# aperezhortal/pySPEEDY

Measured on AMD Instinct MI355X. Metric: simulated-years/day (whole node), T30L8, higher is better.
Workload: dtype f64

## Files before the change

### pyspeedy_amd/csrc/dynamics.hip

```cpp
#include <hip/hip_runtime.h>

#include <type_traits>

#include "coupler_point.hpp"
#include "device_tables.hpp"
#include "diagnostics_block.hpp"
#include "dyn_column.hpp"
#include "launch_events.hpp"
#include "model.hpp"
#include "sppt_point.hpp"

namespace spd {

namespace {
using d2 = double __attribute__((ext_vector_type(2)));
constexpr int NG = IX * IL;
constexpr int kT = 256;

__device__ constexpr double CPd = 1004.0f;
__device__ constexpr double AKAPd = 2.0f / 7.0f;
__device__ constexpr double RGASd = AKAPd * CPd;
__device__ constexpr double WILd = 0.53f, TDRSd = 24.0f * 30.0f;

__device__ inline d2 times_i(d2 z) { return d2{-z.y, z.x}; }
__device__ inline d2 operator_scale(double c, d2 z) { return d2{c * z.x, c * z.y}; }

struct Stencil {
    d2 ac, bc, ap, bp, an, bn;
};
__device__ inline Stencil load_stencil(const d2 *a, const d2 *b, int k, int n) {
    const int kp = n > 0 ? k - MX : k, kn = n < NX - 1 ? k + MX : k;
    return Stencil{a[k], b[k], a[kp], b[kp], a[kn], b[kn]};
}
template <int MODE>
__device__ inline void apply_stencil(const Stencil &s, int k, int m, int n, const DeviceTables &T, d2 &ra, d2 &rb) {
    const double *tym = MODE == 0 ? T.uvdym : T.vddym, *typ = MODE == 0 ? T.uvdyp : T.vddyp;
    const double dx = MODE == 0 ? T.uvdx[k] : T.gradx[m];
    const double cm = tym[k], cp = typ[k];
    const d2 zp = times_i(d2{dx * s.ac.x, dx * s.ac.y}), zc = times_i(d2{dx * s.bc.x, dx * s.bc.y});
    if (n == 0) {
        ra = d2{zc.x - cp * s.an.x, zc.y - cp * s.an.y};
        rb = d2{zp.x + cp * s.bn.x, zp.y + cp * s.bn.y};
    } else if (n == NX - 1) {
        ra = d2{cm * s.ap.x, cm * s.ap.y};
        rb = d2{-cm * s.bp.x, -cm * s.bp.y};
    } else {
        ra = d2{cm * s.ap.x - cp * s.an.x + zc.x, cm * s.ap.y - cp * s.an.y + zc.y};
        rb = d2{-cm * s.bp.x + cp * s.bn.x + zp.x, -cm * s.bp.y + cp * s.bn.y + zp.y};
    }
}
}

namespace {
__device__ __forceinline__ d2 geo_up(d2 ph_below, d2 t_below, d2 t_here, double xg2_below, double xg1_here) {
    return d2{fma(xg1_here, t_here.x, fma(xg2_below, t_below.x, ph_below.x)),
              fma(xg1_here, t_here.y, fma(xg2_below, t_below.y, ph_below.y))};
}
__device__ __forceinline__ d2 geo_corr(d2 ph, d2 t_below, d2 t_above, double corf) {
    return d2{fma(corf, t_below.x - t_above.x, ph.x), fma(corf, t_below.y - t_above.y, ph.y)};
}
}

template <bool SPPT>
__global__ __launch_bounds__(kT) void geopotential_kernel(ModelPtrs P, DynDeviceTables D, int first, int count, int tl, SpptArgs sp) {
    const int ngeo = (count * NSPEC + kT - 1) / kT;
    if (SPPT && static_cast<int>(blockIdx.x) >= ngeo) {
        sppt_update_point(sp, static_cast<long>(blockIdx.x - ngeo) * kT + threadIdx.x);
        return;
    }
    const int gid = blockIdx.x * kT + threadIdx.x;
    if (gid >= count * NSPEC) return;
    const int lm = gid / NSPEC, mem = first + lm, k = gid - lm * NSPEC, m = k % MX;
    const d2 *t = reinterpret_cast<const d2 *>(P.t) + (static_cast<size_t>(mem) * 2 + tl) * 8 * NSPEC + k;
    d2 *phi = reinterpret_cast<d2 *>(P.phi) + static_cast<size_t>(mem) * 8 * NSPEC + k;
    d2 tt[KX], ph[KX];
#pragma unroll
    for (int l = 0; l < KX; ++l) tt[l] = t[static_cast<size_t>(l) * NSPEC];
    const d2 phis = reinterpret_cast<const d2 *>(P.phis)[static_cast<size_t>(mem) * NSPEC + k];
    ph[KX - 1] = d2{fma(D.xgeop1[KX - 1], tt[KX - 1].x, phis.x), fma(D.xgeop1[KX - 1], tt[KX - 1].y, phis.y)};
#pragma unroll
    for (int l = KX - 2; l >= 0; --l) ph[l] = geo_up(ph[l + 1], tt[l + 1], tt[l], D.xgeop2[l + 1], D.xgeop1[l]);
    if (m == 0) {
#pragma unroll
        for (int l = 1; l < KX - 1; ++l) ph[l] = geo_corr(ph[l], tt[l + 1], tt[l - 1], D.geo_corf[l]);
    }
#pragma unroll
    for (int l = 0; l < KX; ++l) phi[static_cast<size_t>(l) * NSPEC] = ph[l];
}

__global__ __launch_bounds__(kT) void dyn_grid_kernel(ModelPtrs P, DynDeviceTables D, int M) {
    const int gid = blockIdx.x * kT + threadIdx.x;
    if (gid >= M * NG) return;
    const int mem = gid / NG, p = gid - mem * NG, j = p / IX;
    double ttend[KX], trtend[KX], ut, vt;
    dyn_column<true>(P, D, mem, p, j, ttend, trtend, ut, vt);
}

namespace {
constexpr int kCoefBlocks = NSPEC / 8;
static_assert(NSPEC % 8 == 0, "coefficient blocks");

__device__ inline void gather_levels(d2 v, int kk, d2 (&out)[KX]) {
#pragma unroll
    for (int l = 0; l < KX; ++l) out[l] = d2{__shfl(v.x, 8 * l + kk), __shfl(v.y, 8 * l + kk)};
}
template <int N>
__device__ inline double pick(const double (&a)[N], int l) {
    double r = a[0];
#pragma unroll
    for (int i = 1; i < N; ++i) r = (l == i) ? a[i] : r;
    return r;
}
template <int N>
__device__ inline d2 pick(const d2 (&a)[N], int l) {
    d2 r = a[0];
#pragma unroll
    for (int i = 1; i < N; ++i) r = (l == i) ? a[i] : r;
    return r;
}
}

struct NoCoupler {};
template <bool FOLD, bool EARLY, typename CA>
__global__ __launch_bounds__(kT) void spectral_step_kernel(ModelPtrs P, DeviceTables T, DynDeviceTables D, int M, int first,
                                                           int count, int j1, double dt, double eps, CA cpl) {
    int nblocks = gridDim.x;
    if constexpr (std::is_same<CA, CouplerArgs>::value) {
        nblocks = (count * NSPEC * KX + kT - 1) / kT;
        if (static_cast<int>(blockIdx.x) >= nblocks) {
            const int gid = (blockIdx.x - nblocks) * kT + threadIdx.x;
            if (gid < cpl.count * NG) {
                const int lm = gid / NG;
                coupler_point(cpl.S, cpl.first + lm, gid - lm * NG, cpl.w, cpl.day, cpl.land_coupling, cpl.sst_anomaly,
                              cpl.anom_planes, cpl.fresh);
            }
            return;
        }
    }
    const int xcd = blockIdx.x & 7, q = nblocks >> 3, r = nblocks & 7;
    const int block = xcd * q + (xcd < r ? xcd : r) + (blockIdx.x >> 3);
    const int gid = block * kT + threadIdx.x;
    const int w = gid >> 6, lane = gid & 63;
    if (w >= count * kCoefBlocks) return;
    const int l = lane >> 3, kk = lane & 7;
    const int lm = w / kCoefBlocks, mem = first + lm, k = (w - lm * kCoefBlocks) * 8 + kk, n = k / MX, m = k - n * MX;
    const size_t f8 = static_cast<size_t>(mem) * 8 * NSPEC;
    const size_t pair = static_cast<size_t>(M) * 8 * NSPEC;
    const size_t fo = static_cast<size_t>(l) * NSPEC;
    const d2 *su = reinterpret_cast<const d2 *>(P.specu) + f8 + fo, *sv = reinterpret_cast<const d2 *>(P.specv) + f8 + fo;
    const double el2 = T.el2[k];
    d2 vordt, divdt, tdt, trdt, dump;
    const size_t s0 = static_cast<size_t>(mem) * 2 * 8 * NSPEC + fo + k;
    const size_t lvl = static_cast<size_t>(8) * NSPEC;
    d2 *vorS = reinterpret_cast<d2 *>(P.vor) + s0, *divS = reinterpret_cast<d2 *>(P.div) + s0;
    d2 *tS = reinterpret_cast<d2 *>(P.t) + s0, *trS = reinterpret_cast<d2 *>(P.tr) + s0;
    d2 *psS = reinterpret_cast<d2 *>(P.ps) + static_cast<size_t>(mem) * 2 * NSPEC + k;
    const int l_tot = m + n;
    d2 ke, stt, str, psdt, ph, div1, ps1;
    d2 vor1, t1, tr1, tcorh, qcorh, phis_k{0.0, 0.0}, vor2{}, div2{}, t2{}, tr2{}, ps2{};
    double xc_l[KX], xj_l[KX], xd_l[KX], elz, dmp, dmp1, dmpd, dmp1d, dmps, dmp1s, trf;
    auto load_diffusion = [&]() {
        dmp = D.dmp[k], dmp1 = D.dmp1[k], dmpd = D.dmpd[k], dmp1d = D.dmp1d[k], dmps = D.dmps[k], dmp1s = D.dmp1s[k];
        trf = T.trfilt[k];
        tcorh = reinterpret_cast<const d2 *>(P.tcorh)[static_cast<size_t>(mem) * NSPEC + k];
        qcorh = reinterpret_cast<const d2 *>(P.qcorh)[static_cast<size_t>(mem) * NSPEC + k];
    };
    if constexpr (EARLY) {
        const Stencil s_uv = load_stencil(su, sv, k, n);
        const Stencil s_ut = load_stencil(su + pair, sv + pair, k, n);
        const Stencil s_uq = load_stencil(su + 2 * pair, sv + 2 * pair, k, n);
        ke = reinterpret_cast<const d2 *>(P.spec_ke)[f8 + fo + k];
        stt = reinterpret_cast<const d2 *>(P.spec_tt)[f8 + fo + k];
        str = reinterpret_cast<const d2 *>(P.spec_tr)[f8 + fo + k];
        psdt = reinterpret_cast<const d2 *>(P.spec_ps)[static_cast<size_t>(mem) * NSPEC + k];
        ph = reinterpret_cast<const d2 *>(P.phi)[f8 + fo + k];
        div1 = divS[0];
        ps1 = psS[0];
        const double *xj = D.xj + static_cast<size_t>(KX) * KX * (l_tot > 0 ? l_tot - 1 : 0);
#pragma unroll
        for (int k1 = 0; k1 < KX; ++k1) xc_l[k1] = D.xc[l + KX * k1], xj_l[k1] = xj[l + KX * k1], xd_l[k1] = D.xd[l + KX * k1];
        elz = D.elz[k];
        load_diffusion();
        vor1 = vorS[0], t1 = tS[0], tr1 = trS[0];
        vor2 = vorS[lvl], div2 = divS[lvl], t2 = tS[lvl], tr2 = trS[lvl], ps2 = psS[NSPEC];
        if (FOLD) phis_k = reinterpret_cast<const d2 *>(P.phis)[static_cast<size_t>(mem) * NSPEC + k];
        apply_stencil<1>(s_uv, k, m, n, T, vordt, divdt);
        const d2 lap = d2{-ke.x * el2, -ke.y * el2};
        divdt = d2{divdt.x - lap.x, divdt.y - lap.y};
        apply_stencil<1>(s_ut, k, m, n, T, dump, tdt);
        tdt = d2{tdt.x + stt.x, tdt.y + stt.y};
        apply_stencil<1>(s_uq, k, m, n, T, dump, trdt);
        trdt = d2{trdt.x + str.x, trdt.y + str.y};
    } else {
        const Stencil s_uv = load_stencil(su, sv, k, n);
        const Stencil s_ut = load_stencil(su + pair, sv + pair, k, n);
        const Stencil s_uq = load_stencil(su + 2 * pair, sv + 2 * pair, k, n);
        ke = reinterpret_cast<const d2 *>(P.spec_ke)[f8 + fo + k];
        stt = reinterpret_cast<const d2 *>(P.spec_tt)[f8 + fo + k];
        str = reinterpret_cast<const d2 *>(P.spec_tr)[f8 + fo + k];
        apply_stencil<1>(s_uv, k, m, n, T, vordt, divdt);
        const d2 lap = d2{-ke.x * el2, -ke.y * el2};
        divdt = d2{divdt.x - lap.x, divdt.y - lap.y};
        apply_stencil<1>(s_ut, k, m, n, T, dump, tdt);
        tdt = d2{tdt.x + stt.x, tdt.y + stt.y};
        apply_stencil<1>(s_uq, k, m, n, T, dump, trdt);
        trdt = d2{trdt.x + str.x, trdt.y + str.y};
        psdt = reinterpret_cast<const d2 *>(P.spec_ps)[static_cast<size_t>(mem) * NSPEC + k];
        div1 = divS[0];
        ps1 = psS[0];
    }
    if (k == 0) psdt = d2{0.0, 0.0};

    const double tref_l = pick(D.tref, l);

    d2 dmeanc{0.0, 0.0};
    {
        d2 dall[KX];
        gather_levels(div1, kk, dall);
#pragma unroll
        for (int j = 0; j < KX; ++j) dmeanc = d2{dmeanc.x + dall[j].x * D.dhs[j], dmeanc.y + dall[j].y * D.dhs[j]};
        psdt = d2{psdt.x - dmeanc.x, psdt.y - dmeanc.y};
        if (k == 0) psdt = d2{0.0, 0.0};
        d2 sig_l{0.0, 0.0}, sig_l1{0.0, 0.0};
#pragma unroll
        for (int j = 0; j < KX - 1; ++j) {
            const d2 term = d2{D.dhs[j] * (dall[j].x - dmeanc.x), D.dhs[j] * (dall[j].y - dmeanc.y)};
            if (j < l) sig_l = d2{sig_l.x - term.x, sig_l.y - term.y};
            if (j <= l) sig_l1 = d2{sig_l1.x - term.x, sig_l1.y - term.y};
        }
        if (l == KX - 1) sig_l1 = d2{0.0, 0.0};
        double dtr_l = 0.0, dtr_l1 = 0.0;
#pragma unroll
        for (int j = 1; j < KX; ++j) {
            const double d = D.tref[j] - D.tref[j - 1];
            dtr_l = (l == j) ? d : dtr_l;
            dtr_l1 = (l + 1 == j) ? d : dtr_l1;
        }
        const d2 dumk_l = d2{sig_l.x * dtr_l, sig_l.y * dtr_l}, dumk_l1 = d2{sig_l1.x * dtr_l1, sig_l1.y * dtr_l1};
        const double dhsr_l = pick(D.dhsr, l), tref3_l = pick(D.tref3, l), tref2_l = pick(D.tref2, l);
        tdt.x = tdt.x - (dumk_l1.x + dumk_l.x) * dhsr_l + tref3_l * (sig_l1.x + sig_l.x) - tref2_l * dmeanc.x;
        tdt.y = tdt.y - (dumk_l1.y + dumk_l.y) * dhsr_l + tref3_l * (sig_l1.y + sig_l.y) - tref2_l * dmeanc.y;
    }
    {
        if constexpr (!EARLY) ph = reinterpret_cast<const d2 *>(P.phi)[f8 + fo + k];
        const double c = RGASd * tref_l;
        const d2 x = d2{ph.x + c * ps1.x, ph.y + c * ps1.y};
        const d2 lap = d2{-x.x * el2, -x.y * el2};
        divdt = d2{divdt.x - lap.x, divdt.y - lap.y};
    }

    {
        d2 all[KX];
        gather_levels(tdt, kk, all);
        d2 ye{0.0, 0.0};
#pragma unroll
        for (int k1 = 0; k1 < KX; ++k1) {
            const double x = EARLY ? xd_l[k1] : D.xd[l + KX * k1];
            ye = d2{ye.x + x * all[k1].x, ye.y + x * all[k1].y};
        }
        if constexpr (!EARLY) elz = D.elz[k];
        const double c = RGASd * tref_l;
        ye = d2{ye.x + c * psdt.x, ye.y + c * psdt.y};
        const d2 yf = d2{divdt.x + elz * ye.x, divdt.y + elz * ye.y};
        divdt = d2{0.0, 0.0};
        gather_levels(yf, kk, all);
        if (l_tot != 0) {
            const double *xj = D.xj + static_cast<size_t>(KX) * KX * (l_tot - 1);
#pragma unroll
            for (int k1 = 0; k1 < KX; ++k1) {
                const double x = EARLY ? xj_l[k1] : xj[l + KX * k1];
                divdt = d2{divdt.x + x * all[k1].x, divdt.y + x * all[k1].y};
            }
        }
        gather_levels(divdt, kk, all);
#pragma unroll
        for (int j = 0; j < KX; ++j) psdt = d2{psdt.x - all[j].x * D.dhsx[j], psdt.y - all[j].y * D.dhsx[j]};
#pragma unroll
        for (int k1 = 0; k1 < KX; ++k1) {
            const double x = EARLY ? xc_l[k1] : D.xc[l + KX * k1];
            tdt = d2{tdt.x + x * all[k1].x, tdt.y + x * all[k1].y};
        }
    }

    if constexpr (!EARLY) load_diffusion();
    const double sdrag = 1.0f / (TDRSd * 3600.0f);
    auto diffuse = [](d2 field, d2 fdt, double a, double b) { return d2{(fdt.x - a * field.x) * b, (fdt.y - a * field.y) * b}; };
    auto advance = [&](d2 *base, size_t stride, d2 o1, d2 o2, d2 fdt) -> d2 {
        if (!EARLY) o1 = base[0], o2 = base[stride];
        fdt = d2{fdt.x * trf, fdt.y * trf};
        const d2 oj = (j1 == 0) ? o1 : o2;
        const d2 fnew = d2{o1.x + dt * fdt.x, o1.y + dt * fdt.y};
        const double we = WILd * eps;
        const d2 n1 = d2{oj.x + we * (o1.x - 2 * oj.x + fnew.x), oj.y + we * (o1.y - 2 * oj.y + fnew.y)};
        const d2 oja = (j1 == 0) ? n1 : oj;
        const double we2 = (1.0f - WILd) * eps;
        const d2 n2 = d2{fnew.x - we2 * (n1.x - 2.0f * oja.x + fnew.x), fnew.y - we2 * (n1.y - 2.0f * oja.y + fnew.y)};
        stream_store(&base[0], n1);
        stream_store(&base[stride], n2);
        return n1;
    };
    {
        if constexpr (!EARLY) vor1 = vorS[0], t1 = tS[0], tr1 = trS[0];
        d2 vd = diffuse(vor1, vordt, dmp, dmp1);
        d2 dd = diffuse(div1, divdt, dmpd, dmp1d);
        const double tcorv_l = pick(D.tcorv, l), qcorv_l = pick(D.qcorv, l);
        const d2 ct = d2{t1.x + tcorh.x * tcorv_l, t1.y + tcorh.y * tcorv_l};
        d2 td = diffuse(ct, tdt, dmp, dmp1);
        if (l == 0 && m == 0) {
            vd = d2{vd.x - sdrag * vor1.x, vd.y - sdrag * vor1.y};
            dd = d2{dd.x - sdrag * div1.x, dd.y - sdrag * div1.y};
        }
        vd = diffuse(vor1, vd, dmps, dmp1s);
        dd = diffuse(div1, dd, dmps, dmp1s);
        td = diffuse(ct, td, dmps, dmp1s);
        const d2 cq = d2{tr1.x + qcorh.x * qcorv_l, tr1.y + qcorh.y * qcorv_l};
        const d2 qd = diffuse(cq, trdt, dmpd, dmp1d);
        advance(vorS, lvl, vor1, vor2, vd);
        advance(divS, lvl, div1, div2, dd);
        const d2 t_new = advance(tS, lvl, t1, t2, td);
        advance(trS, lvl, tr1, tr2, qd);
        if (FOLD) {
            d2 tall[KX];
            gather_levels(t_new, kk, tall);
            if constexpr (!EARLY) phis_k = reinterpret_cast<const d2 *>(P.phis)[static_cast<size_t>(mem) * NSPEC + k];
            d2 pn = d2{fma(D.xgeop1[KX - 1], tall[KX - 1].x, phis_k.x), fma(D.xgeop1[KX - 1], tall[KX - 1].y, phis_k.y)};
#pragma unroll
            for (int j = KX - 2; j >= 0; --j) {
                const d2 up = geo_up(pn, tall[j + 1], tall[j], D.xgeop2[j + 1], D.xgeop1[j]);
                pn = (j >= l) ? up : pn;
            }
            if (m == 0 && l >= 1 && l < KX - 1) {
                d2 tb = tall[2], ta = tall[0];
                double corf = D.geo_corf[1];
#pragma unroll
                for (int j = 2; j < KX - 1; ++j) {
                    tb = (l == j) ? tall[j + 1] : tb;
                    ta = (l == j) ? tall[j - 1] : ta;
                    corf = (l == j) ? D.geo_corf[j] : corf;
                }
                pn = geo_corr(pn, tb, ta, corf);
            }
            stream_store(&reinterpret_cast<d2 *>(P.phi_next)[f8 + fo + k], pn);
        }
    }
    if (l == 0) advance(psS, NSPEC, ps1, ps2, psdt);
}

__global__ __launch_bounds__(64 * KX) void diagnostics_kernel(CheckArgs c, DeviceTables T) {
    diagnostics_block(c, T, c.first + static_cast<int>(blockIdx.x));
}

hipError_t run_geopotential(const ModelPtrs &P, const DynDeviceTables &D, int first, int count, int tl, const SpptArgs *sppt,
                            hipStream_t s) {
    const int ngeo = (count * NSPEC + kT - 1) / kT;
    if (sppt) {
        const long n = static_cast<long>(sppt->M) * KX * NSPEC;
        launch(geopotential_kernel<true>, dim3(ngeo + static_cast<unsigned>((n + kT - 1) / kT)), dim3(kT), 0, s, P, D,
                           first, count, tl, *sppt);
    } else {
        launch(geopotential_kernel<false>, dim3(ngeo), dim3(kT), 0, s, P, D, first, count, tl, SpptArgs{});
    }
    return hipGetLastError();
}
hipError_t run_dyn_grid(const ModelPtrs &P, const DynDeviceTables &D, int M, hipStream_t s) {
    launch(dyn_grid_kernel, dim3((M * NG + kT - 1) / kT), dim3(kT), 0, s, P, D, M);
    return hipGetLastError();
}
namespace {
template <bool FOLD, bool EARLY, typename CA>
void launch_spectral_step(dim3 grid, hipStream_t s, const ModelPtrs &P, const DeviceTables &T, const DynDeviceTables &D, int M,
                          int first, int count, int j1, double dt, double eps, const CA &cpl) {
    launch(spectral_step_kernel<FOLD, EARLY, CA>, grid, dim3(kT), 0, s, P, T, D, M, first, count, j1, dt, eps, cpl);
}
template <typename CA>
void dispatch_spectral_step(bool fold, bool early, dim3 grid, hipStream_t s, const ModelPtrs &P, const DeviceTables &T,
                            const DynDeviceTables &D, int M, int first, int count, int j1, double dt, double eps, const CA &cpl) {
    if (fold && early) launch_spectral_step<true, true, CA>(grid, s, P, T, D, M, first, count, j1, dt, eps, cpl);
    else if (fold) launch_spectral_step<true, false, CA>(grid, s, P, T, D, M, first, count, j1, dt, eps, cpl);
    else if (early) launch_spectral_step<false, true, CA>(grid, s, P, T, D, M, first, count, j1, dt, eps, cpl);
    else launch_spectral_step<false, false, CA>(grid, s, P, T, D, M, first, count, j1, dt, eps, cpl);
}
}
hipError_t run_spectral_step(const ModelPtrs &P, const DeviceTables &T, const DynDeviceTables &D, int M, int first, int count,
                             int j1, double dt, double eps, const CouplerArgs *cpl, bool early, hipStream_t s) {
    const int nspec = (count * NSPEC * KX + kT - 1) / kT;
    const bool fold = P.phi_next != nullptr;
    if (cpl)
        dispatch_spectral_step(fold, early, dim3(nspec + (cpl->count * NG + kT - 1) / kT), s, P, T, D, M, first, count, j1, dt, eps,
                               *cpl);
    else
        dispatch_spectral_step(fold, early, dim3(nspec), s, P, T, D, M, first, count, j1, dt, eps, NoCoupler{});
    return hipGetLastError();
}
hipError_t run_diagnostics(const ModelPtrs &P, const DeviceTables &T, int M, int tl, int *err, double *diag, int ticket,
                           hipStream_t s) {
    hipLaunchKernelGGL(diagnostics_kernel, dim3(M), dim3(64 * KX), 0, s, CheckArgs{P.vor, P.div, P.t, tl, err, diag, ticket}, T);
    return hipGetLastError();
}
hipError_t run_diagnostics_range(const ModelPtrs &P, const DeviceTables &T, int first, int count, int tl, int *err, double *diag,
                                 int ticket, hipStream_t s) {
    if (count <= 0) return hipSuccess;
    hipLaunchKernelGGL(diagnostics_kernel, dim3(count), dim3(64 * KX), 0, s, CheckArgs{P.vor, P.div, P.t, tl, err, diag, ticket, first}, T);
    return hipGetLastError();
}

}
```

### pyspeedy_amd/csrc/model.hip

```cpp
#include <dlfcn.h>
#include <hip/hip_runtime.h>

#include <algorithm>
#include <atomic>
#include <chrono>
#include <cmath>
#include <cstring>
#include <map>
#include <memory>
#include <mutex>
#include <string>
#include <thread>
#include <utility>
#include <vector>

#include "../../include/pyspeedy_amd.h"
#include "context.hpp"
#include "model.hpp"
#include "coupler_point.hpp"
#include "diagnostics_block.hpp"
#include "bounded_call.hpp"
#include "launch_events.hpp"
#include "sppt_point.hpp"
#include "plev.hpp"
// ... 311 lines not shown

static int ensure_tables32(spd_model *m) {
    TableBatch batch;
    if (!m->inv_table32[0][0]) build_inverse_tables(m, false, true, m->inv_table32, batch);
    if (m->sppt_spec && !m->inv_table_sppt32[0][0]) build_inverse_tables(m, true, true, m->inv_table_sppt32, batch);
    return batch.upload(m);
}

static int build_tables(spd_model *m) {
    const int M = m->M;
    const ModelPtrs &P = m->P;
    auto spec = [](double *base, size_t field) { return base + field * NSPEC * C; };
    auto grid = [](double *base, size_t field) { return base + field * NG; };
    TableBatch batch;
    build_inverse_tables(m, false, false, m->inv_table, batch);
    std::vector<FieldDesc> t;
    t.reserve(static_cast<size_t>(M) * 73);
    const size_t pair = static_cast<size_t>(M) * 8;
    for (int i = 0; i < M; ++i) {
        const size_t w = static_cast<size_t>(i) * 8;
        for (int k = 0; k < 8; ++k) {
            t.push_back({grid(P.utend, w + k), spec(P.specu, w + k), 1, 0});
            t.push_back({grid(P.vtend, w + k), spec(P.specv, w + k), 1, 0});
            t.push_back({grid(P.utg, w + k), spec(P.specu, pair + w + k), 1, 0});
            t.push_back({grid(P.vtg, w + k), spec(P.specv, pair + w + k), 1, 0});
            t.push_back({grid(P.uqg, w + k), spec(P.specu, 2 * pair + w + k), 1, 0});
            t.push_back({grid(P.vqg, w + k), spec(P.specv, 2 * pair + w + k), 1, 0});
            t.push_back({grid(P.ttend, w + k), spec(P.spec_tt, w + k), 0, 0});
            t.push_back({grid(P.trtend, w + k), spec(P.spec_tr, w + k), 0, 0});
            t.push_back({grid(P.keg, w + k), spec(P.spec_ke, w + k), 0, 0});
        }
        t.push_back({grid(P.psdtg, i), spec(P.spec_ps, i), 0, 0});
    }
    batch.add(std::move(t), &m->fwd_table);
    for (int par = 0; par < 2; ++par) {
        std::vector<FieldDesc> ti, tf;
        const size_t half = static_cast<size_t>(M) * 16;
        for (int i = 0; i < M; ++i) {
            const size_t w = static_cast<size_t>(i) * 8, s1 = static_cast<size_t>(i) * 16;
            for (int k = 0; k < 8; ++k) {
                ti.push_back({spec(P.sv, s1 + k), grid(m->u_grid, w + k), 2, 0});
                ti.push_back({spec(P.sv, half + s1 + k), grid(m->v_grid, w + k), 2, 0});
                ti.push_back({spec(P.t, s1 + k), grid(m->t_grid, w + k), 1, 0});
                ti.push_back({spec(P.tr, s1 + k), grid(m->q_grid, w + k), 1, 0});
                ti.push_back({spec(m->phi_buf[par], w + k), grid(m->phi_grid, w + k), 1, 0});
                tf.push_back({grid(m->u_grid, w + k), spec(P.sv, s1 + k), 1, 0});
                tf.push_back({grid(m->v_grid, w + k), spec(P.sv, half + s1 + k), 1, 0});
                tf.push_back({grid(m->t_grid, w + k), spec(P.t, s1 + k), 0, 0});
                tf.push_back({grid(m->q_grid, w + k), spec(P.tr, s1 + k), 0, 0});
                tf.push_back({grid(m->phi_grid, w + k), spec(m->phi_buf[par], w + k), 0, 0});
            }
            ti.push_back({spec(P.ps, static_cast<size_t>(i) * 2), grid(m->ps_grid, i), 1, 0});
        }
        batch.add(std::move(ti), &m->exp_inv_table[par]);
        batch.add(std::move(tf), &m->exp_fwd_table[par]);
    }
    return batch.upload(m);
}

extern "C" {

constexpr size_t kMaxDynSteps = 64;
static int dyn_upload(spd_context *ctx, spd_dyn_tables &set, const spd_dyn_tables *base, double *slab) {
    const DynHostTables &dh = set.host;
    DynDeviceTables &D = set.dev;
    std::vector<double> packed;
    auto put = [&](const std::vector<double> &v) {
        const double *at = slab + packed.size();
        packed.insert(packed.end(), v.begin(), v.end());
        return at;
    };
    if (!base) {
        D.dmp = put(dh.dmp); D.dmpd = put(dh.dmpd); D.dmps = put(dh.dmps);
        D.coriol = put(std::vector<double>(ctx->host.coriol.begin(), ctx->host.coriol.end()));
        for (int k = 0; k < 8; ++k) {
            D.tcorv[k] = dh.tcorv[k]; D.qcorv[k] = dh.qcorv[k]; D.tref[k] = dh.tref[k]; D.tref2[k] = dh.tref2[k];
            D.tref3[k] = dh.tref3[k]; D.xgeop1[k] = dh.xgeop1[k]; D.xgeop2[k] = dh.xgeop2[k]; D.geo_corf[k] = dh.geo_corf[k];
            D.dhs[k] = ctx->host.dhs[k]; D.dhsr[k] = ctx->host.dhsr[k]; D.fsgr[k] = ctx->host.fsgr[k];
        }
    } else {
        D = base->dev;
        D.dmp1 = put(dh.dmp1); D.dmp1d = put(dh.dmp1d); D.dmp1s = put(dh.dmp1s); D.elz = put(dh.elz); D.xj = put(dh.xj);
        D.xc = put(std::vector<double>(dh.xc.begin(), dh.xc.end()));
        D.xd = put(std::vector<double>(dh.xd.begin(), dh.xd.end()));
        for (int k = 0; k < 8; ++k) D.dhsx[k] = dh.dhsx[k];
    }
    M_HIP(hipMemcpy(slab, packed.data(), packed.size() * sizeof(double), hipMemcpyHostToDevice));
    return SPD_OK;
}
constexpr size_t kDynSlabDoubles = 4 * NSPEC + 8 * 8 * (MX + NX + 1) + 128;

static int dyn_tables(spd_context *ctx, double dt, spd_model *owner, const spd_dyn_tables **out) {
    std::lock_guard<std::mutex> lock(ctx->dyn_mutex);
    M_HIP(hipSetDevice(ctx->device));
    auto slab = [&](double **p) -> int {
        void *d = nullptr;
        M_HIP(hipMalloc(&d, kDynSlabDoubles * sizeof(double)));
        ctx->allocations.push_back(d);
        *p = static_cast<double *>(d);
        return SPD_OK;
    };
    if (!ctx->dyn_base) {
        auto base = std::make_unique<spd_dyn_tables>(DynHostTables(ctx->host));
        double *d = nullptr;
        if (int rc = slab(&d)) return rc;
        if (int rc = dyn_upload(ctx, *base, nullptr, d)) return rc;
        ctx->dyn_base = std::move(base);
    }
    if (dt == 0.0) {
        *out = ctx->dyn_base.get();
        return SPD_OK;
    }
    auto it = ctx->dyn_by_step.find(dt);
    if (it != ctx->dyn_by_step.end()) {
        *out = it->second.get();
        return SPD_OK;
    }
    auto set = std::make_unique<spd_dyn_tables>(ctx->dyn_base->host);
    set->host.set_time_step(ctx->host, dt);
    if (ctx->dyn_by_step.size() < kMaxDynSteps) {
        double *d = nullptr;
        if (int rc = slab(&d)) return rc;
        if (int rc = dyn_upload(ctx, *set, ctx->dyn_base.get(), d)) return rc;
        *out = set.get();
        ctx->dyn_by_step.emplace(dt, std::move(set));
        return SPD_OK;
    }
    if (!owner) return m_fail(SPD_E_ARG, "dyn_tables: the context holds its maximum of time steps");
    double *d = owner->dyn_private ? const_cast<double *>(owner->dyn_private->dev.dmp1) : nullptr;
    if (!d) {
        void *p = nullptr;
        if (int rc = arena_alloc(owner, kDynSlabDoubles * sizeof(double), &p)) return rc;
        d = static_cast<double *>(p);
    }
    M_HIP(hipDeviceSynchronize());
    if (int rc = dyn_upload(ctx, *set, ctx->dyn_base.get(), d)) return rc;
    owner->dyn_private = std::move(set);
    *out = owner->dyn_private.get();
    return SPD_OK;
}

int spd_model_create(spd_handle h, int nmembers, spd_model_handle *out) {
    if (!h || !out) return m_fail(SPD_E_ARG, "spd_model_create: null argument");
    if (nmembers <= 0) return m_fail(SPD_E_ARG, "spd_model_create: nmembers must be positive");
    *out = nullptr;
    M_HIP(hipSetDevice(h->device));
    spd_model *m = new spd_model();
    m->ctx = h;
    m->M = nmembers;
    if (const char *env = getenv("PYSPEEDY_AMD_SPLIT_DYN")) m->split_dyn_physics = atoi(env) != 0;
    m->inv_per_member = 77;
    if (const char *env = getenv("PYSPEEDY_AMD_PRUNE_DEAD")) m->inv_per_member = atoi(env) != 0 ? 77 : 91;
    if (const char *env = getenv("PYSPEEDY_AMD_DIAG_EVERY_STEP")) m->diag_every_step = atoi(env) != 0;
    m->fold_geo = nmembers <= 8;
    if (const char *env = getenv("PYSPEEDY_AMD_SPECTRAL_EARLY")) m->spectral_early = atoi(env);
    if (const char *env = getenv("PYSPEEDY_AMD_FOLD_GEO")) m->fold_geo = atoi(env) != 0;
    if (const char *env = getenv("PYSPEEDY_AMD_PHYS_STORE32")) m->phys_store32 = atoi(env) != 0;
    m->nchunks = nmembers >= 64 ? 2 : (nmembers >= 24 ? 3 : (nmembers >= 20 ? 2 : 1));
    if (const char *env = getenv("PYSPEEDY_AMD_CHUNKS")) m->nchunks = atoi(env);
    if (m->nchunks < 1) m->nchunks = 1;
    if (m->nchunks > 4) m->nchunks = 4;
    if (m->nchunks > nmembers) m->nchunks = nmembers;
    if (const char *env = getenv("PYSPEEDY_AMD_BLOCK_MEMBERS")) m->block_members = atoi(env) > 0 ? atoi(env) : 0;
    const size_t M = nmembers, S = NSPEC * C, G3 = static_cast<size_t>(8) * NG;
    ModelPtrs &P = m->P;
    spd_physics_args &pa = m->pa;
    int rc = SPD_OK;
#define A(ptr, doubles, name, per)                      \
    if (rc == SPD_OK) rc = dalloc(m, (doubles), &(ptr), name, (per) * sizeof(double))
    A(P.vor, M * 2 * 8 * S, "vor", 2 * 8 * S);
    A(P.div, M * 2 * 8 * S, "div", 2 * 8 * S);
    A(P.t, M * 2 * 8 * S, "t", 2 * 8 * S);
    A(P.tr, M * 2 * 8 * S, "tr", 2 * 8 * S);
    A(P.ps, M * 2 * S, "ps", 2 * S);
    A(P.phi, M * 8 * S, "phi", 8 * S);
    A(m->phi_buf[1], M * 8 * S, nullptr, 0);
    m->phi_buf[0] = P.phi;
    A(P.phis, M * S, "phis", S);
    A(P.tcorh, M * S, "tcorh", S);
    A(P.qcorh, M * S, "qcorh", S);
    A(P.sv, 4 * M * 8 * S, nullptr, 0);
    A(P.vorg, M * G3, nullptr, 0); A(P.divg, M * G3, nullptr, 0); A(P.tg2, M * G3, nullptr, 0);
    A(P.trg2, M * G3, nullptr, 0); A(P.ug2, M * G3, nullptr, 0); A(P.vg2, M * G3, nullptr, 0);
    A(P.px, M * NG, nullptr, 0); A(P.py, M * NG, nullptr, 0);
    A(P.utend, M * G3, nullptr, 0); A(P.vtend, M * G3, nullptr, 0); A(P.ttend, M * G3, nullptr, 0);
    A(P.trtend, M * G3, nullptr, 0); A(P.keg, M * G3, nullptr, 0); A(P.utg, M * G3, nullptr, 0);
    A(P.vtg, M * G3, nullptr, 0); A(P.uqg, M * G3, nullptr, 0); A(P.vqg, M * G3, nullptr, 0);
    A(P.psdtg, M * NG, nullptr, 0);
    A(P.specu, 3 * M * 8 * S, nullptr, 0); A(P.specv, 3 * M * 8 * S, nullptr, 0);
    A(P.spec_tt, M * 8 * S, nullptr, 0); A(P.spec_tr, M * 8 * S, nullptr, 0); A(P.spec_ke, M * 8 * S, nullptr, 0);
    A(P.spec_ps, M * S, nullptr, 0);
    double *tmp = nullptr;
#define PA_IN(field, doubles, name, per)                            \
    A(tmp, doubles, name, per);                                     \
    pa.field = tmp
    PA_IN(ug, M * G3, "u_grid_phys", G3); PA_IN(vg, M * G3, "v_grid_phys", G3); PA_IN(tg, M * G3, "t_grid_phys", G3);
    PA_IN(qg, M * G3, "q_grid_phys", G3); PA_IN(phig, M * G3, "phi_grid_phys", G3); PA_IN(pslg, M * NG, "pslg_phys", NG);
    pa.utend = P.utend; pa.vtend = P.vtend; pa.ttend = P.ttend; pa.qtend = P.trtend;
#define PA2(field) PA_IN(field, M * NG, #field, NG)
    PA2(fmask_land); PA2(phis0); PA2(forog); PA2(sst_am); PA2(alb_land); PA2(alb_sea); PA2(snowc); PA2(land_temp);
    PA2(soil_avail_water); PA2(flux_solar_in); PA2(flux_ozone_upper); PA2(flux_ozone_lower); PA2(zenit_correction);
    PA2(stratospheric_correction); PA2(alb_surface);
    PA2(precnv); PA2(precls); PA2(cbmf); PA2(slrd); PA2(slr); PA2(olr); PA2(tsr); PA2(ssrd); PA2(ssr); PA2(qcloud_equiv);
#define PA3(field) PA_IN(field, M * 3 * NG, #field, 3 * NG)
    PA3(slru); PA3(ustr); PA3(vstr); PA3(shf); PA3(evap); PA3(hfluxn);
    PA_IN(rad_st4a, M * 2 * G3, "rad_st4a", 2 * G3);
    PA_IN(rad_flux, M * 4 * NG, "rad_flux", 4 * NG);
    PA_IN(tt_rsw, M * G3, "tt_rsw", G3);
    PA_IN(rad_tau2, M * 4 * G3, "rad_tau2", 4 * G3);
    PA_IN(rad_strat_corr, M * 2 * NG, "rad_strat_corr", 2 * NG);
    SurfacePtrs &SF = m->S;
    const size_t G12 = static_cast<size_t>(12) * NG;
    A(SF.stl12, M * G12, "stl12", G12); A(SF.snowd12, M * G12, "snowd12", G12); A(SF.soilw12, M * G12, "soilw12", G12);
    A(SF.sst12, M * G12, "sst12", G12); A(SF.sea_ice_frac12, M * G12, "sea_ice_frac12", G12);
    A(SF.sst_anom, M * 3 * NG, "sst_anom", 3 * NG);
    A(m->soil_wc_l1, M * G12, "soil_wc_l1", G12); A(m->soil_wc_l2, M * G12, "soil_wc_l2", G12);
    A(m->soil_wc_l3, M * G12, "soil_wc_l3", G12);
#define S2(field) A(SF.field, M * NG, #field, NG)
    S2(stlcl_obs); S2(snowdcl_obs); S2(soilwcl_obs); S2(stl_lm); S2(snow_depth); S2(cdland); S2(rhcapl);
    S2(sstcl_ob); S2(sicecl_ob); S2(ticecl_ob); S2(sstan_ob); S2(sst_om); S2(tice_om); S2(sice_om); S2(sstan_am);
    S2(sice_am); S2(tice_am); S2(ssti_om); S2(cdsea); S2(cdice); S2(rhcaps); S2(rhcapi); S2(hfseacl); S2(fmask_sea);
#undef S2
    A(tmp, M * NG, "alb0", NG); SF.alb0 = tmp;
    A(m->orog, M * NG, "orog", NG); A(m->phi0, M * NG, "phi0", NG); A(m->fmask_orig, M * NG, "fmask_orig", NG);
    A(m->veg_high, M * NG, "veg_high", NG); A(m->veg_low, M * NG, "veg_low", NG);
    A(m->bmask_land, M * NG, "bmask_land", NG); A(m->bmask_sea, M * NG, "bmask_sea", NG);
    A(m->u_grid, M * G3, "u_grid", G3); A(m->v_grid, M * G3, "v_grid", G3); A(m->t_grid, M * G3, "t_grid", G3);
    A(m->q_grid, M * G3, "q_grid", G3); A(m->phi_grid, M * G3, "phi_grid", G3); A(m->ps_grid, M * NG, "ps_grid", NG);
    A(m->corh_t, M * NG, nullptr, 0); A(m->corh_q, M * NG, nullptr, 0); A(m->scratch_spec, 2 * M * S, nullptr, 0);
    SF.land_temp = const_cast<double *>(pa.land_temp); SF.soil_avail_water = const_cast<double *>(pa.soil_avail_water);
    SF.sst_am = const_cast<double *>(pa.sst_am); SF.hfluxn = pa.hfluxn; SF.shf = pa.shf; SF.evap = pa.evap; SF.ssrd = pa.ssrd;
    SF.flux_solar_in = const_cast<double *>(pa.flux_solar_in); SF.flux_ozone_upper = const_cast<double *>(pa.flux_ozone_upper);
    SF.flux_ozone_lower = const_cast<double *>(pa.flux_ozone_lower); SF.zenit_correction = const_cast<double *>(pa.zenit_correction);
    SF.stratospheric_correction = const_cast<double *>(pa.stratospheric_correction);
    SF.snowc = const_cast<double *>(pa.snowc); SF.alb_land = const_cast<double *>(pa.alb_land);
    SF.alb_sea = const_cast<double *>(pa.alb_sea); SF.alb_surface = const_cast<double *>(pa.alb_surface);
    SF.fmask_land = pa.fmask_land; SF.phis0 = pa.phis0;
#undef PA3
#undef PA2
#undef PA_IN
#undef A
    if (rc != SPD_OK) {
        spd_model_destroy(m);
        return rc;
    }
    for (const char *name : {"t_grid_phys", "q_grid_phys", "phi_grid_phys", "pslg_phys", "u_grid_phys", "v_grid_phys",
                             "tt_rsw", "rad_tau2", "rad_strat_corr",
                             "rad_st4a", "rad_flux", "precnv", "precls", "cbmf", "slrd", "slr", "olr", "slru", "ustr", "vstr"})
        m->reg[name].f32 = true;
    if (rc == SPD_OK) {
        const spd_dyn_tables *base = nullptr;
        rc = dyn_tables(h, 0.0, nullptr, &base);
        if (rc == SPD_OK) m->D = base->dev;
    }
    if (rc == SPD_OK) {
        void *p = nullptr;
        rc = arena_alloc(m, sizeof(int) * M, &p);
        m->d_err = static_cast<int *>(p);
        if (rc == SPD_OK) rc = arena_alloc(m, sizeof(double) * M * 24, &p);
        m->d_diag = static_cast<double *>(p);
    }
    if (rc == SPD_OK) rc = build_tables(m);
    if (rc != SPD_OK) {
        spd_model_destroy(m);
        return rc;
    }
    *out = m;
    return SPD_OK;
}

int spd_model_destroy(spd_model_handle m) {
    if (!m) return SPD_OK;
    (void)hipSetDevice(m->ctx->device);
    constexpr size_t kIdleBytes = static_cast<size_t>(1) << 30;
    bool keep_first = false;
    if (!m->blocks.empty() && hipDeviceSynchronize() == hipSuccess) {
        std::lock_guard<std::mutex> lock(m->ctx->idle_mutex);
        if (m->ctx->idle_bytes + m->blocks[0].size <= kIdleBytes) {
            m->ctx->idle_blocks.push_back({m->blocks[0].base, m->blocks[0].size});
            m->ctx->idle_bytes += m->blocks[0].size;
            keep_first = true;
        }
    }
    for (size_t i = keep_first ? 1 : 0; i < m->blocks.size(); ++i) (void)hipFree(m->blocks[i].base);
    for (int i = 0; i < 4; ++i) {
        if (m->cstream[i]) (void)hipStreamDestroy(m->cstream[i]);
        if (m->cev[i]) (void)hipEventDestroy(m->cev[i]);
    }
    if (m->stats.alloc) (void)hipFree(m->stats.alloc);
    if (m->ev_start) (void)hipEventDestroy(m->ev_start);
    if (m->ev_offset) (void)hipEventDestroy(m->ev_offset);
    if (m->h_err_sync) (void)hipHostFree(m->h_err_sync);
    if (m->h_steps_err) (void)hipHostFree(m->h_steps_err);
    if (m->steps_event) (void)hipEventDestroy(m->steps_event);
    for (int i = 0; i < 2; ++i) {
        if (m->h_err[i]) (void)hipHostFree(m->h_err[i]);
        if (m->err_event[i]) (void)hipEventDestroy(m->err_event[i]);
    }
    for (auto &pr : m->prof_events) {
        (void)hipEventDestroy(pr.first);
        (void)hipEventDestroy(pr.second);
    }
    delete m;
    return SPD_OK;
}

int spd_model_members(spd_model_handle m) { return m ? m->M : SPD_E_ARG; }
// ... 1699 lines not shown
```

Before: 1.685 million.

## Restructure spectral step loads with uniform offsets, phased scheduling, and default geo folding

Reworks address computation in the non-early spectral step so a wave-uniform base pointer plus a 32-bit per-lane offset is used, with readfirstlane on the wave index. Loads are regrouped into phases separated by scheduling barriers, and plain stores replace streaming stores. Occupancy hints are added to launch bounds, and geopotential folding is enabled for all member counts. The intent is to cut address arithmetic and VGPR pressure and to overlap loads better, at the cost of tighter register limits and a different schedule for large ensembles.

New measurement: 1.683 million (median of 3 runs). About the same (-0.1%).

```diff
diff --git a/pyspeedy_amd/csrc/dynamics.hip b/pyspeedy_amd/csrc/dynamics.hip
--- a/pyspeedy_amd/csrc/dynamics.hip
+++ b/pyspeedy_amd/csrc/dynamics.hip
@@ -31,6 +31,15 @@
 __device__ inline Stencil load_stencil(const d2 *a, const d2 *b, int k, int n) {
     const int kp = n > 0 ? k - MX : k, kn = n < NX - 1 ? k + MX : k;
     return Stencil{a[k], b[k], a[kp], b[kp], a[kn], b[kn]};
+}
+template <bool UNIFORM, typename T>
+__device__ __forceinline__ T *elem(T *base, size_t u, unsigned v) {
+    if constexpr (UNIFORM) return (T *)((const char *)(base + u) + v * static_cast<unsigned>(sizeof(T)));
+    else return base + (u + v);
+}
+__device__ inline Stencil load_stencil_at(const d2 *a, const d2 *b, unsigned oc, unsigned op, unsigned on) {
+    return Stencil{*elem<true>(a, 0, oc), *elem<true>(b, 0, oc), *elem<true>(a, 0, op),
+                   *elem<true>(b, 0, op), *elem<true>(a, 0, on), *elem<true>(b, 0, on)};
 }
 template <int MODE>
 __device__ inline void apply_stencil(const Stencil &s, int k, int m, int n, const DeviceTables &T, d2 &ra, d2 &rb) {
@@ -122,8 +131,9 @@
 
 struct NoCoupler {};
 template <bool FOLD, bool EARLY, typename CA>
-__global__ __launch_bounds__(kT) void spectral_step_kernel(ModelPtrs P, DeviceTables T, DynDeviceTables D, int M, int first,
-                                                           int count, int j1, double dt, double eps, CA cpl) {
+__global__ __launch_bounds__(kT, EARLY ? 2 : 4) void spectral_step_kernel(ModelPtrs P, DeviceTables T, DynDeviceTables D, int M,
+                                                                           int first, int count, int j1, double dt, double eps,
+                                                                           CA cpl) {
     int nblocks = gridDim.x;
     if constexpr (std::is_same<CA, CouplerArgs>::value) {
         nblocks = (count * NSPEC * KX + kT - 1) / kT;
@@ -140,7 +150,7 @@
     const int xcd = blockIdx.x & 7, q = nblocks >> 3, r = nblocks & 7;
     const int block = xcd * q + (xcd < r ? xcd : r) + (blockIdx.x >> 3);
     const int gid = block * kT + threadIdx.x;
-    const int w = gid >> 6, lane = gid & 63;
+    const int w = EARLY ? gid >> 6 : __builtin_amdgcn_readfirstlane(gid >> 6), lane = gid & 63;
     if (w >= count * kCoefBlocks) return;
     const int l = lane >> 3, kk = lane & 7;
     const int lm = w / kCoefBlocks, mem = first + lm, k = (w - lm * kCoefBlocks) * 8 + kk, n = k / MX, m = k - n * MX;
@@ -150,40 +160,48 @@
     const d2 *su = reinterpret_cast<const d2 *>(P.specu) + f8 + fo, *sv = reinterpret_cast<const d2 *>(P.specv) + f8 + fo;
     const double el2 = T.el2[k];
     d2 vordt, divdt, tdt, trdt, dump;
-    const size_t s0 = static_cast<size_t>(mem) * 2 * 8 * NSPEC + fo + k;
+    constexpr bool U = !EARLY;
+    unsigned o8 = static_cast<unsigned>(l * NSPEC + k), ok = static_cast<unsigned>(k);
+    auto new_phase = [&]() {
+        if constexpr (U) asm volatile("" : "+v"(o8), "+v"(ok));
+    };
+    const size_t s0 = static_cast<size_t>(mem) * 2 * 8 * NSPEC;
     const size_t lvl = static_cast<size_t>(8) * NSPEC;
-    d2 *vorS = reinterpret_cast<d2 *>(P.vor) + s0, *divS = reinterpret_cast<d2 *>(P.div) + s0;
-    d2 *tS = reinterpret_cast<d2 *>(P.t) + s0, *trS = reinterpret_cast<d2 *>(P.tr) + s0;
-    d2 *psS = reinterpret_cast<d2 *>(P.ps) + static_cast<size_t>(mem) * 2 * NSPEC + k;
+    const size_t f1 = static_cast<size_t>(mem) * NSPEC;
+    auto state = [&](double *base, int tl) { return elem<U>(reinterpret_cast<d2 *>(base), s0 + tl * lvl, o8); };
+    auto ps_at = [&](int tl) { return elem<U>(reinterpret_cast<d2 *>(P.ps), 2 * f1 + tl * NSPEC, ok); };
+    auto work8 = [&](const double *base) { return elem<U>(reinterpret_cast<const d2 *>(base), f8, o8); };
+    auto field1 = [&](const double *base) { return elem<U>(reinterpret_cast<const d2 *>(base), f1, ok); };
+    auto coef = [&](const double *table) { return *elem<U>(table, 0, ok); };
     const int l_tot = m + n;
     d2 ke, stt, str, psdt, ph, div1, ps1;
     d2 vor1, t1, tr1, tcorh, qcorh, phis_k{0.0, 0.0}, vor2{}, div2{}, t2{}, tr2{}, ps2{};
     double xc_l[KX], xj_l[KX], xd_l[KX], elz, dmp, dmp1, dmpd, dmp1d, dmps, dmp1s, trf;
     auto load_diffusion = [&]() {
-        dmp = D.dmp[k], dmp1 = D.dmp1[k], dmpd = D.dmpd[k], dmp1d = D.dmp1d[k], dmps = D.dmps[k], dmp1s = D.dmp1s[k];
-        trf = T.trfilt[k];
-        tcorh = reinterpret_cast<const d2 *>(P.tcorh)[static_cast<size_t>(mem) * NSPEC + k];
-        qcorh = reinterpret_cast<const d2 *>(P.qcorh)[static_cast<size_t>(mem) * NSPEC + k];
+        dmp = coef(D.dmp), dmp1 = coef(D.dmp1), dmpd = coef(D.dmpd), dmp1d = coef(D.dmp1d), dmps = coef(D.dmps), dmp1s = coef(D.dmp1s);
+        trf = coef(T.trfilt);
+        tcorh = *field1(P.tcorh);
+        qcorh = *field1(P.qcorh);
     };
     if constexpr (EARLY) {
         const Stencil s_uv = load_stencil(su, sv, k, n);
         const Stencil s_ut = load_stencil(su + pair, sv + pair, k, n);
         const Stencil s_uq = load_stencil(su + 2 * pair, sv + 2 * pair, k, n);
-        ke = reinterpret_cast<const d2 *>(P.spec_ke)[f8 + fo + k];
-        stt = reinterpret_cast<const d2 *>(P.spec_tt)[f8 + fo + k];
-        str = reinterpret_cast<const d2 *>(P.spec_tr)[f8 + fo + k];
-        psdt = reinterpret_cast<const d2 *>(P.spec_ps)[static_cast<size_t>(mem) * NSPEC + k];
-        ph = reinterpret_cast<const d2 *>(P.phi)[f8 + fo + k];
-        div1 = divS[0];
-        ps1 = psS[0];
+        ke = *work8(P.spec_ke);
+        stt = *work8(P.spec_tt);
+        str = *work8(P.spec_tr);
+        psdt = *field1(P.spec_ps);
+        ph = *work8(P.phi);
+        div1 = *state(P.div, 0);
+        ps1 = *ps_at(0);
         const double *xj = D.xj + static_cast<size_t>(KX) * KX * (l_tot > 0 ? l_tot - 1 : 0);
 #pragma unroll
         for (int k1 = 0; k1 < KX; ++k1) xc_l[k1] = D.xc[l + KX * k1], xj_l[k1] = xj[l + KX * k1], xd_l[k1] = D.xd[l + KX * k1];
-        elz = D.elz[k];
+        elz = coef(D.elz);
         load_diffusion();
-        vor1 = vorS[0], t1 = tS[0], tr1 = trS[0];
-        vor2 = vorS[lvl], div2 = divS[lvl], t2 = tS[lvl], tr2 = trS[lvl], ps2 = psS[NSPEC];
-        if (FOLD) phis_k = reinterpret_cast<const d2 *>(P.phis)[static_cast<size_t>(mem) * NSPEC + k];
+        vor1 = *state(P.vor, 0), t1 = *state(P.t, 0), tr1 = *state(P.tr, 0);
+        vor2 = *state(P.vor, 1), div2 = *state(P.div, 1), t2 = *state(P.t, 1), tr2 = *state(P.tr, 1), ps2 = *ps_at(1);
+        if (FOLD) phis_k = *field1(P.phis);
         apply_stencil<1>(s_uv, k, m, n, T, vordt, divdt);
         const d2 lap = d2{-ke.x * el2, -ke.y * el2};
         divdt = d2{divdt.x - lap.x, divdt.y - lap.y};
@@ -192,12 +210,21 @@
         apply_stencil<1>(s_uq, k, m, n, T, dump, trdt);
         trdt = d2{trdt.x + str.x, trdt.y + str.y};
     } else {
-        const Stencil s_uv = load_stencil(su, sv, k, n);
-        const Stencil s_ut = load_stencil(su + pair, sv + pair, k, n);
-        const Stencil s_uq = load_stencil(su + 2 * pair, sv + 2 * pair, k, n);
-        ke = reinterpret_cast<const d2 *>(P.spec_ke)[f8 + fo + k];
-        stt = reinterpret_cast<const d2 *>(P.spec_tt)[f8 + fo + k];
-        str = reinterpret_cast<const d2 *>(P.spec_tr)[f8 + fo + k];
+        const int kp = n > 0 ? k - MX : k, kn = n < NX - 1 ? k + MX : k;
+        const unsigned op = static_cast<unsigned>(l * NSPEC + kp), on = static_cast<unsigned>(l * NSPEC + kn);
+        const d2 *u0 = reinterpret_cast<const d2 *>(P.specu) + f8, *v0 = reinterpret_cast<const d2 *>(P.specv) + f8;
+        const Stencil s_uv = load_stencil_at(u0, v0, o8, op, on);
+        const Stencil s_ut = load_stencil_at(u0 + pair, v0 + pair, o8, op, on);
+        const Stencil s_uq = load_stencil_at(u0 + 2 * pair, v0 + 2 * pair, o8, op, on);
+        ke = *work8(P.spec_ke);
+        stt = *work8(P.spec_tt);
+        str = *work8(P.spec_tr);
+        psdt = *field1(P.spec_ps);
+        ph = *work8(P.phi);
+        div1 = *state(P.div, 0);
+        ps1 = *ps_at(0);
+        elz = coef(D.elz);
+        __builtin_amdgcn_sched_barrier(0);
         apply_stencil<1>(s_uv, k, m, n, T, vordt, divdt);
         const d2 lap = d2{-ke.x * el2, -ke.y * el2};
         divdt = d2{divdt.x - lap.x, divdt.y - lap.y};
@@ -205,9 +232,10 @@
         tdt = d2{tdt.x + stt.x, tdt.y + stt.y};
         apply_stencil<1>(s_uq, k, m, n, T, dump, trdt);
         trdt = d2{trdt.x + str.x, trdt.y + str.y};
-        psdt = reinterpret_cast<const d2 *>(P.spec_ps)[static_cast<size_t>(mem) * NSPEC + k];
-        div1 = divS[0];
-        ps1 = psS[0];
+        new_phase();
+        __builtin_amdgcn_sched_barrier(0);
+        vor2 = *state(P.vor, 1), div2 = *state(P.div, 1), t2 = *state(P.t, 1), tr2 = *state(P.tr, 1), ps2 = *ps_at(1);
+        __builtin_amdgcn_sched_barrier(0);
     }
     if (k == 0) psdt = d2{0.0, 0.0};
 
@@ -242,7 +270,6 @@
         tdt.y = tdt.y - (dumk_l1.y + dumk_l.y) * dhsr_l + tref3_l * (sig_l1.y + sig_l.y) - tref2_l * dmeanc.y;
     }
     {
-        if constexpr (!EARLY) ph = reinterpret_cast<const d2 *>(P.phi)[f8 + fo + k];
         const double c = RGASd * tref_l;
         const d2 x = d2{ph.x + c * ps1.x, ph.y + c * ps1.y};
         const d2 lap = d2{-x.x * el2, -x.y * el2};
@@ -258,7 +285,6 @@
             const double x = EARLY ? xd_l[k1] : D.xd[l + KX * k1];
             ye = d2{ye.x + x * all[k1].x, ye.y + x * all[k1].y};
         }
-        if constexpr (!EARLY) elz = D.elz[k];
         const double c = RGASd * tref_l;
         ye = d2{ye.x + c * psdt.x, ye.y + c * psdt.y};
         const d2 yf = d2{divdt.x + elz * ye.x, divdt.y + elz * ye.y};
@@ -282,11 +308,22 @@
         }
     }
 
-    if constexpr (!EARLY) load_diffusion();
+    if constexpr (!EARLY) {
+        asm volatile("" : "+v"(psdt.x), "+v"(psdt.y));
+        new_phase();
+        __builtin_amdgcn_sched_barrier(0);
+        vor1 = *state(P.vor, 0), t1 = *state(P.t, 0), tr1 = *state(P.tr, 0);
+        load_diffusion();
+        if (FOLD) phis_k = *field1(P.phis);
+        __builtin_amdgcn_sched_barrier(0);
+    }
     const double sdrag = 1.0f / (TDRSd * 3600.0f);
+    auto put = [](d2 *p, d2 v) {
+        if constexpr (EARLY) stream_store(p, v);
+        else *p = v;
+    };
     auto diffuse = [](d2 field, d2 fdt, double a, double b) { return d2{(fdt.x - a * field.x) * b, (fdt.y - a * field.y) * b}; };
-    auto advance = [&](d2 *base, size_t stride, d2 o1, d2 o2, d2 fdt) -> d2 {
-        if (!EARLY) o1 = base[0], o2 = base[stride];
+    auto advance = [&](d2 *p1, d2 *p2, d2 o1, d2 o2, d2 fdt) -> d2 {
         fdt = d2{fdt.x * trf, fdt.y * trf};
         const d2 oj = (j1 == 0) ? o1 : o2;
         const d2 fnew = d2{o1.x + dt * fdt.x, o1.y + dt * fdt.y};
@@ -295,12 +332,11 @@
         const d2 oja = (j1 == 0) ? n1 : oj;
         const double we2 = (1.0f - WILd) * eps;
         const d2 n2 = d2{fnew.x - we2 * (n1.x - 2.0f * oja.x + fnew.x), fnew.y - we2 * (n1.y - 2.0f * oja.y + fnew.y)};
-        stream_store(&base[0], n1);
-        stream_store(&base[stride], n2);
+        put(p1, n1);
+        put(p2, n2);
         return n1;
     };
     {
-        if constexpr (!EARLY) vor1 = vorS[0], t1 = tS[0], tr1 = trS[0];
         d2 vd = diffuse(vor1, vordt, dmp, dmp1);
         d2 dd = diffuse(div1, divdt, dmpd, dmp1d);
         const double tcorv_l = pick(D.tcorv, l), qcorv_l = pick(D.qcorv, l);
@@ -315,14 +351,15 @@
         td = diffuse(ct, td, dmps, dmp1s);
         const d2 cq = d2{tr1.x + qcorh.x * qcorv_l, tr1.y + qcorh.y * qcorv_l};
         const d2 qd = diffuse(cq, trdt, dmpd, dmp1d);
-        advance(vorS, lvl, vor1, vor2, vd);
-        advance(divS, lvl, div1, div2, dd);
-        const d2 t_new = advance(tS, lvl, t1, t2, td);
-        advance(trS, lvl, tr1, tr2, qd);
+        new_phase();
+        advance(state(P.vor, 0), state(P.vor, 1), vor1, vor2, vd);
+        advance(state(P.div, 0), state(P.div, 1), div1, div2, dd);
+        const d2 t_new = advance(state(P.t, 0), state(P.t, 1), t1, t2, td);
+        advance(state(P.tr, 0), state(P.tr, 1), tr1, tr2, qd);
+        if (l == 0) advance(ps_at(0), ps_at(1), ps1, ps2, psdt);
         if (FOLD) {
             d2 tall[KX];
             gather_levels(t_new, kk, tall);
-            if constexpr (!EARLY) phis_k = reinterpret_cast<const d2 *>(P.phis)[static_cast<size_t>(mem) * NSPEC + k];
             d2 pn = d2{fma(D.xgeop1[KX - 1], tall[KX - 1].x, phis_k.x), fma(D.xgeop1[KX - 1], tall[KX - 1].y, phis_k.y)};
 #pragma unroll
             for (int j = KX - 2; j >= 0; --j) {
@@ -340,10 +377,10 @@
                 }
                 pn = geo_corr(pn, tb, ta, corf);
             }
-            stream_store(&reinterpret_cast<d2 *>(P.phi_next)[f8 + fo + k], pn);
-        }
-    }
-    if (l == 0) advance(psS, NSPEC, ps1, ps2, psdt);
+            new_phase();
+            put(elem<U>(reinterpret_cast<d2 *>(P.phi_next), f8, o8), pn);
+        }
+    }
 }
 
 __global__ __launch_bounds__(64 * KX) void diagnostics_kernel(CheckArgs c, DeviceTables T) {
diff --git a/pyspeedy_amd/csrc/model.hip b/pyspeedy_amd/csrc/model.hip
--- a/pyspeedy_amd/csrc/model.hip
+++ b/pyspeedy_amd/csrc/model.hip
@@ -487,7 +487,7 @@
     m->inv_per_member = 77;
     if (const char *env = getenv("PYSPEEDY_AMD_PRUNE_DEAD")) m->inv_per_member = atoi(env) != 0 ? 77 : 91;
     if (const char *env = getenv("PYSPEEDY_AMD_DIAG_EVERY_STEP")) m->diag_every_step = atoi(env) != 0;
-    m->fold_geo = nmembers <= 8;
+    m->fold_geo = true;
     if (const char *env = getenv("PYSPEEDY_AMD_SPECTRAL_EARLY")) m->spectral_early = atoi(env);
     if (const char *env = getenv("PYSPEEDY_AMD_FOLD_GEO")) m->fold_geo = atoi(env) != 0;
     if (const char *env = getenv("PYSPEEDY_AMD_PHYS_STORE32")) m->phys_store32 = atoi(env) != 0;
```
